# apple/ml-neuman

Hardware: AMD Instinct MI355X
Metric: rays_per_sec (800x800 frame, 128 samples/ray coarse + 128 importance, NeuMan background NeRF) (higher is better)
Workload: dtype coarse (sampling) pass: split-fp16 hi+lo MFMA x3, f32 accumulate; fine (shading) pass: per-row-scaled int16 as two int8 limbs on the i8 MFMA x3, exact int32 accumulate, encodings on split bf16

## Files before the change

### ml-neuman_amd/csrc/mlp_i8as.h

```cpp
#pragma once
#include "mlp_device.h"

namespace {

typedef __attribute__((ext_vector_type(4))) int i32x4;
typedef __attribute__((ext_vector_type(16))) int i32x16;
typedef __attribute__((ext_vector_type(2))) short i16x2;
typedef __attribute__((address_space(3))) const float lds_cfloat;
typedef __attribute__((ext_vector_type(4))) float vf4;
typedef __attribute__((address_space(3))) const vf4 lds_cvf4;

constexpr int kRows = 32;
struct Args8s {
    MlpArgs a;
    const float* consts8;
    const uint4* image8;
    nm::LiveList live;
};

__device__ __forceinline__ i32x4 as_i32x4(uint4 v) { return __builtin_bit_cast(i32x4, v); }

template <bool F16 = false>
__device__ __forceinline__ void fill_pe_wave(uint4* pw, bool is_dir, const MlpArgs& a, int64_t base_row, int lane) {
    const PeSpec spec = is_dir ? a.dir : a.pos;
    const float* tab = a.petab + (is_dir ? 96 : 0);
    unsigned short* hi = reinterpret_cast<unsigned short*>(pw);
    auto put = [&](int row, int p, float v, bool clamp = false) {
        const int off = ((p >> 3) * (2 * kRows) + row) * 8 + (p & 7);
        if (F16) {
            float sv = v * kF16ActScale;
            if (clamp) sv = __builtin_amdgcn_fmed3f(sv, -65504.f, 65504.f);
            const _Float16 hb = (_Float16)sv;
            const _Float16 lb = (_Float16)(sv - (float)hb);
            hi[off] = __builtin_bit_cast(unsigned short, hb);
            hi[off + kRows * 8] = __builtin_bit_cast(unsigned short, lb);
            return;
        }
        const bf16x2 hb = __builtin_convertvector((f32x2){v, 0.f}, bf16x2);
        const f32x2 hf = __builtin_convertvector(hb, f32x2);
        const bf16x2 lb = __builtin_convertvector((f32x2){v - hf.x, 0.f}, bf16x2);
        hi[off] = (unsigned short)(__builtin_bit_cast(unsigned, hb) & 0xffffu);
        hi[off + kRows * 8] = (unsigned short)(__builtin_bit_cast(unsigned, lb) & 0xffffu);
    };
    if (spec.octaves) {
#pragma unroll 1
        for (int round = 0; round < 2; ++round) {
            const int j = 2 * round + (lane >> 5), row = lane & 31;
            if (j > 2) break;
            int64_t i = base_row + row;
            if (i >= a.n) i = a.n - 1;
            float x0, x1, x2;
            sample_input(a, i, is_dir, x0, x1, x2);
            const float xj = j == 0 ? x0 : (j == 1 ? x1 : x2);
            const float a0 = spec.kind == NM_PE_POSENC ? xj * tab[0] : fmaf(x2, tab[3 * j + 2], fmaf(x1, tab[3 * j + 1], x0 * tab[3 * j]));
            put(row, j, xj);
            double sn, cs;
            sincos_f64((double)a0, sn, cs);
            const int n3 = 3 * spec.nfreq;
            for (int b = 0; b < spec.nfreq; ++b) {
                if (spec.kind == NM_PE_POSENC) { put(row, 3 + 6 * b + j, (float)sn); put(row, 3 + 6 * b + 3 + j, (float)cs); }
                else { put(row, 3 + 3 * b + j, (float)sn); put(row, 3 + n3 + 3 * b + j, (float)cs); }
                const double s2 = 2.0 * sn * cs, c2 = 1.0 - 2.0 * sn * sn;
                sn = s2; cs = c2;
            }
        }
    } else {
        const int nchunks = is_dir ? 4 : nm::kPeChunks;
        for (int item = lane; item < nchunks * kRows; item += 64) {
            const int c = item >> 5, row = item & 31;
            int64_t i = base_row + row;
            if (i >= a.n) i = a.n - 1;
            float x0, x1, x2;
            sample_input(a, i, is_dir, x0, x1, x2);
#pragma unroll
            for (int e = 0; e < 8; ++e) put(row, 8 * c + e, pe_feature(8 * c + e, x0, x1, x2, spec, tab), true);
        }
    }
}

struct X8 {
    uint4 h[8], l[8];
};

__device__ __forceinline__ void glds16(const void* gsrc, unsigned lds_dst) {
    unsigned keep;
    asm volatile("s_mov_b32 %0, m0\n\ts_mov_b32 m0, %2\n\ts_nop 0\n\tglobal_load_lds_dwordx4 %1, off\n\ts_mov_b32 m0, %0"
                 : "=&s"(keep) : "v"(gsrc), "s"(lds_dst) : "memory");
}
__device__ __forceinline__ void bias16(f32x16& f, lds_cfloat* bias_blk) {
#pragma unroll
    for (int q = 0; q < 4; ++q) {
        const vf4 bs = *(lds_cvf4*)(bias_blk + 8 * q);
        f[4 * q] = bs.x; f[4 * q + 1] = bs.y; f[4 * q + 2] = bs.z; f[4 * q + 3] = bs.w;
    }
}
__device__ __forceinline__ void dequant16(f32x16& f, const i32x16& t, float sx256, lds_cfloat* bias_blk) {
#pragma unroll
    for (int q = 0; q < 4; ++q) {
        const vf4 bs = *(lds_cvf4*)(bias_blk + 8 * q);
        const float bsv[4] = {bs.x, bs.y, bs.z, bs.w};
#pragma unroll
        for (int j = 0; j < 4; ++j) f[4 * q + j] = fmaf((float)t[4 * q + j], sx256, bsv[j]);
    }
}
template <bool RELU>
__device__ __forceinline__ float max16(float m, const f32x16& f) {
#pragma unroll
    for (int r = 0; r < 16; ++r) m = fmaxf(m, RELU ? f[r] : fabsf(f[r]));
    return m;
}
__device__ __forceinline__ float row_max(float m) {
    typedef __attribute__((ext_vector_type(2))) unsigned u32x2;
    const u32x2 sw = __builtin_amdgcn_permlane32_swap(__float_as_uint(m), __float_as_uint(m), false, false);
    return fmaxf(__uint_as_float(sw.x), __uint_as_float(sw.y));
}
template <bool RELU>
__device__ __forceinline__ void quant16(const f32x16& f, float inv, uint4& xh, uint4& xl) {
    i16x2 P[8], Y[8];
#pragma unroll
    for (int i = 0; i < 8; ++i) {
        float y0 = f[2 * i] * inv, y1 = f[2 * i + 1] * inv;
        if (RELU) {
            y0 = __builtin_amdgcn_fmed3f(y0, 0.f, 1.f);
            y1 = __builtin_amdgcn_fmed3f(y1, 0.f, 1.f);
        }
        const i16x2 p = __builtin_amdgcn_cvt_pknorm_i16(y0, y1);
        P[i] = p;
        Y[i] = p + (i16x2){128, 128};
    }
    unsigned lo[4], hi[4];
#pragma unroll
    for (int k = 0; k < 4; ++k) {
        lo[k] = __builtin_amdgcn_perm(__builtin_bit_cast(unsigned, P[2 * k + 1]), __builtin_bit_cast(unsigned, P[2 * k]), 0x06040200u);
        hi[k] = __builtin_amdgcn_perm(__builtin_bit_cast(unsigned, Y[2 * k + 1]), __builtin_bit_cast(unsigned, Y[2 * k]), 0x07050301u);
    }
    xh = make_uint4(hi[0], hi[1], hi[2], hi[3]);
    xl = make_uint4(lo[0], lo[1], lo[2], lo[3]);
}
__device__ __forceinline__ float inv_of(float M) { return M > 0.f ? ((float)nm::kFixedMax / 32767.f) * __builtin_amdgcn_rcpf(M) : 0.f; }
__device__ __forceinline__ float scale_of(float M) { return M > 0.f ? M * (1.f / (float)nm::kFixedMax) : 1.f; }

constexpr int kWaves = 8;
constexpr int kTile = kWaves * kRows;
constexpr int kPWaveU4 = nm::kPeChunks * 2 * kRows;
constexpr int kPeU4 = kWaves * kPWaveU4;
constexpr int kStepU4 = nm::kStepBytes / 16;
constexpr int kSlotU4 = 12 * kStepU4;
constexpr int kSlots = 3;
constexpr int kBiasU4 = (nm::kBiasFloats + 16 + 3) / 4;
__host__ __device__ constexpr int block_pieces(int nsteps) { return (2 * nsteps + kWaves - 1) / kWaves; }

template <class S>
struct RingT {
    const char* src;
    const uint4* rd;
    unsigned lds0;
    int off;
    int slot;
    int refill, np, nsteps2;
};
template <class S>
__device__ __forceinline__ void ring_piece(const RingT<S>& R, int off, int slot, int j) {
    glds16(R.src + off + j * (kWaves * 1024), __builtin_amdgcn_readfirstlane(R.lds0 + slot * (kSlotU4 * 16) + j * (kWaves * 1024)));
}
template <class S>
__device__ __forceinline__ void ring_advance(RingT<S>& R, int nsteps) {
    R.off += nsteps * nm::kStepBytes;
    if (R.off == S::kBytes) R.off = 0;
}
template <class S>
__device__ __forceinline__ const uint4* ring_enter(RingT<S>& R, int i) {
    const int np1 = block_pieces(S::steps(i + 1));
    if (np1 == 1) asm volatile("s_waitcnt vmcnt(1)" ::: "memory");
    else if (np1 == 2) asm volatile("s_waitcnt vmcnt(2)" ::: "memory");
    else asm volatile("s_waitcnt vmcnt(3)" ::: "memory");
    __builtin_amdgcn_s_barrier();
    const uint4* cur = R.rd + R.slot * kSlotU4;
    R.refill = R.slot == 0 ? kSlots - 1 : R.slot - 1;
    R.slot = R.slot == kSlots - 1 ? 0 : R.slot + 1;
    R.np = block_pieces(S::steps(i + 2));
    R.nsteps2 = S::steps(i + 2);
    return cur;
}
template <class S>
__device__ __forceinline__ void ring_copy(RingT<S>& R, int j) {
    if (j < R.np) ring_piece(R, R.off, R.refill, j);
    if (j == R.np - 1) ring_advance(R, R.nsteps2);
}
struct W8 {
    uint4 h, l;
};

template <int NSTEPS, bool PEND, bool RELU = true, class Ring>
__device__ __forceinline__ void k_i8_impl(i32x16& t, const X8& X, const uint4* ws, Ring& R, f32x16& fp, const i32x16& tp, lds_cfloat* bias_blk,
                                          float sx256, float& m) {
    i32x16 ah, ac;
#pragma unroll
    for (int r = 0; r < 16; ++r) { ah[r] = 0; ac[r] = 0; }
    W8 w[2];
    w[0].h = ws[0]; w[0].l = ws[64];
    w[1].h = ws[kStepU4]; w[1].l = ws[kStepU4 + 64];
#pragma unroll
    for (int s = 0; s < NSTEPS; ++s) {
        const uint4 wh = w[s & 1].h, wl = w[s & 1].l;
        ac = __builtin_amdgcn_mfma_i32_32x32x32_i8(as_i32x4(wh), as_i32x4(X.l[s]), ac, 0, 0, 0);
        ah = __builtin_amdgcn_mfma_i32_32x32x32_i8(as_i32x4(wh), as_i32x4(X.h[s]), ah, 0, 0, 0);
        ac = __builtin_amdgcn_mfma_i32_32x32x32_i8(as_i32x4(wl), as_i32x4(X.h[s]), ac, 0, 0, 0);
        if (s + 2 < NSTEPS) { w[s & 1].h = ws[(s + 2) * kStepU4]; w[s & 1].l = ws[(s + 2) * kStepU4 + 64]; }
        if (s == 0 || s == 2 || s == 4) ring_copy(R, s >> 1);
        if (PEND) {
            const int r = 2 * s;
            const float b0 = bias_blk[8 * (r >> 2) + (r & 3)], b1 = bias_blk[8 * (r >> 2) + (r & 3) + 1];
            const float f0 = fmaf((float)tp[r], sx256, b0), f1 = fmaf((float)tp[r + 1], sx256, b1);
            fp[r] = f0;
            fp[r + 1] = f1;
            m = RELU ? fmaxf(m, fmaxf(f0, f1)) : fmaxf(m, fmaxf(fabsf(f0), fabsf(f1)));
            __builtin_amdgcn_sched_barrier(0);
        }
    }
#pragma unroll
    for (int r = 0; r < 16; ++r) t[r] = (ah[r] << 8) + ac[r];
}
template <int NSTEPS, class Ring>
__device__ __forceinline__ void k_i8(i32x16& t, const X8& X, const uint4* ws, Ring& R) {
    f32x16 nf;
    float nm_ = 0.f;
    k_i8_impl<NSTEPS, false>(t, X, ws, R, nf, t, nullptr, 0.f, nm_);
}
struct NoRing {};
__device__ __forceinline__ void ring_copy(NoRing&, int) {}
template <int NSTEPS>
struct Enc {
    uint4 h[NSTEPS], l[NSTEPS];
};
template <int NSTEPS>
__device__ __forceinline__ void load_enc(Enc<NSTEPS>& E, const uint4* pw, int g, int s) {
    asm volatile("" ::: "memory");
#pragma unroll
    for (int t = 0; t < NSTEPS; ++t) {
        E.h[t] = pw[(2 * t + g) * (2 * kRows) + s];
        E.l[t] = pw[(2 * t + g) * (2 * kRows) + kRows + s];
    }
}
template <int NSTEPS, bool COPY = false, class Ring = NoRing>
__device__ __forceinline__ void k_bf(f32x16& f, const Enc<NSTEPS>& E, const uint4* ws, Ring* R = nullptr, int j0 = 0) {
#pragma unroll
    for (int t = 0; t < NSTEPS; ++t) {
        if (COPY && (t == 1 || t == 3)) ring_copy(*R, j0 + (t >> 1));
        const uint4 wh = ws[t * kStepU4], wl = ws[t * kStepU4 + 64];
        f = __builtin_amdgcn_mfma_f32_32x32x16_bf16(as_bf16x8(wh), as_bf16x8(E.l[t]), f, 0, 0, 0);
        f = __builtin_amdgcn_mfma_f32_32x32x16_bf16(as_bf16x8(wl), as_bf16x8(E.h[t]), f, 0, 0, 0);
        f = __builtin_amdgcn_mfma_f32_32x32x16_bf16(as_bf16x8(wh), as_bf16x8(E.h[t]), f, 0, 0, 0);
    }
}

}
```

Measured before the change: 1.583 million.

## Split positional-encoding octaves across wave halves with packed vectorized LDS stores

```diff
diff --git a/ml-neuman_amd/csrc/mlp_i8as.h b/ml-neuman_amd/csrc/mlp_i8as.h
--- a/ml-neuman_amd/csrc/mlp_i8as.h
+++ b/ml-neuman_amd/csrc/mlp_i8as.h
@@ -19,6 +19,142 @@
 };
 
 __device__ __forceinline__ i32x4 as_i32x4(uint4 v) { return __builtin_bit_cast(i32x4, v); }
+
+__device__ __forceinline__ void wave_row_input(const MlpArgs& a, int64_t base_row, int row, bool is_dir, float& x0, float& x1, float& x2) {
+    int64_t i = base_row + row;
+    if (i >= a.n) i = a.n - 1;
+    int mode = a.in_mode;
+    unsigned S = (unsigned)a.S;
+    asm volatile("" : "+s"(mode), "+s"(S));
+    if (mode == 0 || mode == 4) {
+        sample_input(a, i, is_dir, x0, x1, x2);
+        return;
+    }
+    int64_t r, zi;
+    if (mode == 3) {
+        const unsigned k = (unsigned)a.ray_idx[i];
+        r = k / S;
+        zi = k;
+    } else {
+        const int64_t i0 = base_row < a.n ? base_row : a.n - 1;
+        const unsigned i0l = __builtin_amdgcn_readfirstlane((unsigned)(uint64_t)i0), i0h = __builtin_amdgcn_readfirstlane((unsigned)((uint64_t)i0 >> 32));
+        const uint64_t u0 = ((uint64_t)i0h << 32) | i0l;
+        const uint64_t q0 = i0h == 0 ? (uint64_t)(i0l / S) : u0 / (uint64_t)S;
+        const unsigned off = (unsigned)(u0 - q0 * S) + (unsigned)(i - i0);
+        const unsigned dq = S >= 32u ? (off >= S ? 1u : 0u) : off / S;
+        const int64_t j = (int64_t)q0 + dq;
+        if (mode != 2) {
+            r = j;
+            zi = i;
+        } else {
+            r = a.ray_idx[j];
+            zi = r * a.S_total + a.s0 + (off - dq * S);
+        }
+    }
+    const float* d = a.direction + r * 3;
+    if (is_dir) {
+        x0 = d[0]; x1 = d[1]; x2 = d[2];
+    } else {
+        const float zz = a.z[zi];
+        const float* o = a.origin + r * 3;
+        x0 = o[0] + d[0] * zz;
+        x1 = o[1] + d[1] * zz;
+        x2 = o[2] + d[2] * zz;
+    }
+}
+
+__device__ __forceinline__ void octave_step(double& sn, double& cs, bool take) {
+    const double s2 = 2.0 * sn * cs, c2 = 1.0 - 2.0 * sn * sn;
+    if (take) { sn = s2; cs = c2; }
+}
+
+template <int F, int END, int BASE, int NP>
+__device__ __forceinline__ void store_run(unsigned short* prow, const unsigned (&P)[NP]) {
+    static_assert((BASE & 1) == 0, "pairs are dwords of the row");
+    if constexpr (F < END) {
+        constexpr int q = F - BASE, m = q >> 1;
+        unsigned short* dst = prow + (F >> 3) * (2 * kRows * 8) + (F & 7);
+        if constexpr ((F & 7) == 0 && END - F >= 8) {
+            *reinterpret_cast<uint4*>(dst) = make_uint4(P[m], P[m + 1], P[m + 2], P[m + 3]);
+            store_run<F + 8, END, BASE>(prow, P);
+        } else if constexpr ((F & 3) == 0 && END - F >= 4) {
+            *reinterpret_cast<uint2*>(dst) = make_uint2(P[m], P[m + 1]);
+            store_run<F + 4, END, BASE>(prow, P);
+        } else if constexpr ((F & 1) == 0 && END - F >= 2) {
+            *reinterpret_cast<unsigned*>(dst) = P[m];
+            store_run<F + 2, END, BASE>(prow, P);
+        } else {
+            *dst = (unsigned short)((q & 1) ? P[m] >> 16 : P[m] & 0xffffu);
+            store_run<F + 1, END, BASE>(prow, P);
+        }
+    }
+}
+
+template <bool F16>
+__device__ __forceinline__ void split_pair(float v0, float v1, unsigned& hp, unsigned& lp) {
+    f32x2 v = {v0, v1};
+    if (F16) {
+        v.x = v.x * kF16ActScale;
+        v.y = v.y * kF16ActScale;
+        const f16x2 hb = __builtin_convertvector(v, f16x2);
+        const f32x2 hf = __builtin_convertvector(hb, f32x2);
+        const f16x2 lb = __builtin_convertvector((f32x2){v.x - hf.x, v.y - hf.y}, f16x2);
+        hp = __builtin_bit_cast(unsigned, hb);
+        lp = __builtin_bit_cast(unsigned, lb);
+    } else {
+        const bf16x2 hb = __builtin_convertvector(v, bf16x2);
+        const f32x2 hf = __builtin_convertvector(hb, f32x2);
+        const bf16x2 lb = __builtin_convertvector((f32x2){v.x - hf.x, v.y - hf.y}, bf16x2);
+        hp = __builtin_bit_cast(unsigned, hb);
+        lp = __builtin_bit_cast(unsigned, lb);
+    }
+}
+
+template <bool F16, int H>
+struct PosencPacked {
+    static constexpr int NQ = 3 + 6 * H, NP = (NQ + 1) / 2, UP = 6 * H;
+    static constexpr int avail(int b) { return b < 0 ? 0 : (b >= H - 1 ? 2 * NP : 9 + 6 * b); }
+    static constexpr int lo_to(int b) { return b < 0 ? 0 : (b >= H - 1 ? NQ : avail(b) & ~7); }
+    static constexpr int up_to(int b) { return b >= H - 1 ? NQ + UP : (b < 0 || ((avail(b) + UP) & ~7) < NQ ? NQ : (avail(b) + UP) & ~7); }
+
+    template <int B>
+    static __device__ __forceinline__ void bands(float (&V)[2 * NP], unsigned (&HP)[NP], unsigned (&LP)[NP], double (&sn)[3], double (&cs)[3],
+                                                 unsigned short* prow, bool up) {
+        if constexpr (B < H) {
+#pragma unroll
+            for (int j = 0; j < 3; ++j) {
+                V[3 + 6 * B + j] = (float)sn[j];
+                V[3 + 6 * B + 3 + j] = (float)cs[j];
+                if (B + 1 < H) octave_step(sn[j], cs[j], true);
+            }
+#pragma unroll
+            for (int m = avail(B - 1) / 2; m < avail(B) / 2; ++m) split_pair<F16>(V[2 * m], V[2 * m + 1], HP[m], LP[m]);
+            if (!up) {
+                store_run<lo_to(B - 1), lo_to(B), 0>(prow, HP);
+                store_run<lo_to(B - 1), lo_to(B), 0>(prow + kRows * 8, LP);
+            } else {
+                store_run<up_to(B - 1), up_to(B), UP>(prow, HP);
+                store_run<up_to(B - 1), up_to(B), UP>(prow + kRows * 8, LP);
+            }
+            bands<B + 1>(V, HP, LP, sn, cs, prow, up);
+        }
+    }
+
+    static __device__ __forceinline__ void run(uint4* pw, float f0, float x0, float x1, float x2, int row, bool up) {
+        float V[2 * NP];
+        unsigned HP[NP], LP[NP];
+        double sn[3], cs[3];
+        V[0] = x0; V[1] = x1; V[2] = x2;
+        V[2 * NP - 1] = 0.f;
+#pragma unroll
+        for (int j = 0; j < 3; ++j) {
+            sincos_f64((double)(V[j] * f0), sn[j], cs[j]);
+#pragma unroll
+            for (int t = 0; t < H; ++t) octave_step(sn[j], cs[j], up);
+        }
+        bands<0>(V, HP, LP, sn, cs, reinterpret_cast<unsigned short*>(pw) + row * 8, up);
+    }
+};
 
 template <bool F16 = false>
 __device__ __forceinline__ void fill_pe_wave(uint4* pw, bool is_dir, const MlpArgs& a, int64_t base_row, int lane) {
@@ -43,25 +179,32 @@
         hi[off + kRows * 8] = (unsigned short)(__builtin_bit_cast(unsigned, lb) & 0xffffu);
     };
     if (spec.octaves) {
+        asm volatile("" : "+v"(lane));
+        const int row = lane & 31;
+        const bool up = lane >= 32;
+        float x0, x1, x2;
+        wave_row_input(a, base_row, row, is_dir, x0, x1, x2);
+        if (spec.kind == NM_PE_POSENC && spec.nfreq == (is_dir ? 4 : 10)) {
+            if (is_dir) PosencPacked<F16, 2>::run(pw, tab[0], x0, x1, x2, row, up);
+            else PosencPacked<F16, 5>::run(pw, tab[0], x0, x1, x2, row, up);
+            return;
+        }
+        const int h = (spec.nfreq + 1) >> 1, n3 = 3 * spec.nfreq;
+        const int first = up ? h : 0, mine = up ? spec.nfreq - h : h;
 #pragma unroll 1
-        for (int round = 0; round < 2; ++round) {
-            const int j = 2 * round + (lane >> 5), row = lane & 31;
-            if (j > 2) break;
-            int64_t i = base_row + row;
-            if (i >= a.n) i = a.n - 1;
-            float x0, x1, x2;
-            sample_input(a, i, is_dir, x0, x1, x2);
+        for (int j = 0; j < 3; ++j) {
             const float xj = j == 0 ? x0 : (j == 1 ? x1 : x2);
             const float a0 = spec.kind == NM_PE_POSENC ? xj * tab[0] : fmaf(x2, tab[3 * j + 2], fmaf(x1, tab[3 * j + 1], x0 * tab[3 * j]));
-            put(row, j, xj);
+            if (!up) put(row, j, xj);
             double sn, cs;
             sincos_f64((double)a0, sn, cs);
-            const int n3 = 3 * spec.nfreq;
-            for (int b = 0; b < spec.nfreq; ++b) {
-                if (spec.kind == NM_PE_POSENC) { put(row, 3 + 6 * b + j, (float)sn); put(row, 3 + 6 * b + 3 + j, (float)cs); }
-                else { put(row, 3 + 3 * b + j, (float)sn); put(row, 3 + n3 + 3 * b + j, (float)cs); }
-                const double s2 = 2.0 * sn * cs, c2 = 1.0 - 2.0 * sn * sn;
-                sn = s2; cs = c2;
+            for (int t = 0; t < 2 * h; ++t) {
+                if (t >= h && t - h < mine) {
+                    const int b = first + t - h;
+                    if (spec.kind == NM_PE_POSENC) { put(row, 3 + 6 * b + j, (float)sn); put(row, 3 + 6 * b + 3 + j, (float)cs); }
+                    else { put(row, 3 + 3 * b + j, (float)sn); put(row, 3 + n3 + 3 * b + j, (float)cs); }
+                }
+                octave_step(sn, cs, t >= h || up);
             }
         }
     } else {
```

Result: no change. 1.594 million (median of 6 runs) (+0.7%).
